# OpenResearchInstitute/opv-cxx-demod

Measured on AMD Instinct MI355X. Metric: IQ Msamples/s demod+Viterbi (×real-time @2.168MSPS); BER vs ref, higher is better.
Workload: dtype f64; 1 GPU; configs[3]: 64 concurrent IQ streams/GPU x 1000 frames, -s semantics, amp 2000, f0 -2000..+2000 Hz across the 64 streams of a shard (SURVEY.md §8d C4: edge streams on the AFC clamp, outside the +/-1530 Hz search span), Eb/N0 16 dB; streams_per_gpu=64, parallelism=streams sharded 64/GPU, no data-path collective

## Files before the change

### opv-cxx-demod_amd/csrc/k_frontend.hip

```cpp
#include <hip/hip_runtime.h>
#include <math.h>

#include <type_traits>

#include "k_frontend_common.h"

namespace {

constexpr uint32_t kTile = OPV_TILE_SAMPLES;
constexpr uint32_t kRing = 2 * kTile;
constexpr uint32_t kRingBytes = kRing * 4;
constexpr uint32_t kGuardBytes = 16;
constexpr uint32_t kBack = 11;
constexpr uint32_t kAhead = 56;
static_assert((kRing & (kRing - 1)) == 0, "ring must be a power of two");

constexpr uint32_t kTabOff = kRingBytes + kGuardBytes;
static_assert(kTabOff % 16 == 0, "16-byte LDS alignment");
constexpr uint32_t kAtanQBytes = 1025 * 32;
constexpr uintptr_t kRbLdsBase = 16;
static_assert(kRbLdsBase + kTabOff + kAtanQBytes == OPV_RB_LDS_I16, "launch size of the int16-ring shape");

constexpr uint32_t kF64Ring = 2048;
constexpr uint32_t kF64RingBytes = kF64Ring * 32;
constexpr uint32_t kF64Chunk = 256;
constexpr uint32_t kF64TabOff = 0;
constexpr uint32_t kF64RingOff = kAtanQBytes;
constexpr uint32_t kF64FlagOff = kF64RingOff + kF64RingBytes;
constexpr uint32_t kF64WaitSpins = 1u << 22;
constexpr uint32_t kHelperSpins = 1u << 22;
static_assert(kRbLdsBase + kF64FlagOff + 16 == OPV_RB_LDS_F64, "launch size of the fp64-ring shape");
static_assert(kF64Ring % kF64Chunk == 0 && (kF64Ring & (kF64Ring - 1)) == 0, "chunks tile the power-of-two ring");

typedef double d2v __attribute__((ext_vector_type(2)));
typedef __attribute__((address_space(3))) unsigned char lbyte;
typedef __attribute__((address_space(3))) int lint;
typedef __attribute__((address_space(3))) double ldouble;
typedef __attribute__((address_space(3))) d2v ld2v;

__device__ inline double swap32_add(double a, double b) {
    auto lo = __builtin_amdgcn_permlane32_swap((unsigned)dlo(a), (unsigned)dlo(b), false, false);
    auto hi = __builtin_amdgcn_permlane32_swap((unsigned)dhi(a), (unsigned)dhi(b), false, false);
    return mkd((int)hi[0], (int)lo[0]) + mkd((int)hi[1], (int)lo[1]);
}
__device__ inline double swap16_add(double a, double b) {
    auto lo = __builtin_amdgcn_permlane16_swap((unsigned)dlo(a), (unsigned)dlo(b), false, false);
    auto hi = __builtin_amdgcn_permlane16_swap((unsigned)dhi(a), (unsigned)dhi(b), false, false);
    return mkd((int)hi[0], (int)lo[0]) + mkd((int)hi[1], (int)lo[1]);
}
template <int N>
__device__ inline double row_bcast(double old, double v) { return __builtin_amdgcn_update_dpp(old, v, 0x150 + N, 0xF, 0xF, false); }
__device__ inline uint32_t uni(uint32_t v) { return (uint32_t)__builtin_amdgcn_readfirstlane((int)v); }
__device__ inline double readlane_d(double v, int l) {
    return mkd(__builtin_amdgcn_readlane(dhi(v), l), __builtin_amdgcn_readlane(dlo(v), l));
}
__device__ inline bool uni_lt(double a, double b) { return __builtin_amdgcn_fcmp(a, b, 4 ) != 0ull; }
__device__ inline bool uni_eq(double a, double b) { return __builtin_amdgcn_fcmp(a, b, 1 ) != 0ull; }

struct TagFirst { static constexpr bool first = true, wide = true; };
struct TagSecond { static constexpr bool first = false, wide = true; };
struct TagSteady { static constexpr bool first = false, wide = false; };

struct SinCosK {
    double s0, s1, s2, s3;
    double c0, c1, c2, c3, c4;
};
__device__ inline void expj_small(double kfs, double fo, const SinCosK& k, double& xs, double& xc) {
    double x, u, p, r, t;
    asm("v_mul_f64 %[x], %[kfs], %[fo]\n\t"
        "v_mul_f64 %[u], %[x], %[x]\n\t"
        "v_fma_f64 %[r], %[c4], %[u], %[c3]\n\t"
        "v_fma_f64 %[p], %[s3], %[u], %[s2]\n\t"
        "v_fma_f64 %[r], %[r], %[u], %[c2]\n\t"
        "v_fma_f64 %[p], %[p], %[u], %[s1]\n\t"
        "v_fma_f64 %[r], %[r], %[u], %[c1]\n\t"
        "v_fma_f64 %[p], %[p], %[u], %[s0]\n\t"
        "v_fma_f64 %[r], %[r], %[u], %[c0]\n\t"
        "v_mul_f64 %[t], %[x], %[u]\n\t"
        "v_fma_f64 %[xc], %[r], %[u], 1.0\n\t"
        "v_fma_f64 %[xs], %[t], %[p], %[x]"
        : [x] "=&v"(x), [u] "=&v"(u), [p] "=&v"(p), [r] "=&v"(r), [t] "=&v"(t), [xs] "=&v"(xs), [xc] "=&v"(xc)
        : [kfs] "v"(kfs), [fo] "v"(fo), [s0] "v"(k.s0), [s1] "v"(k.s1), [s2] "v"(k.s2), [s3] "v"(k.s3),
          [c0] "v"(k.c0), [c1] "v"(k.c1), [c2] "v"(k.c2), [c3] "v"(k.c3), [c4] "v"(k.c4));
}

}

#include "opv_atan2.h"

typedef __attribute__((address_space(3))) volatile uint32_t lds_flag;
__device__ inline lds_flag* f64_flags(lbyte* lds_all) {
    return reinterpret_cast<lds_flag*>(lds_all + kF64FlagOff);
}

__device__ void f64_ring_helper(const OpvStream& st, lbyte* lds_all) {
    const uint32_t lane = threadIdx.x & 63u;
    lds_flag* const fl = f64_flags(lds_all);
    const uint32_t n_avail = uni((uint32_t)st.n_avail), origin = uni((uint32_t)st.origin);
    const int* const iq = reinterpret_cast<const int*>(st.iq);
    uint32_t fill = ((origin >= kBack ? origin - kBack : 0u) / kF64Chunk) * kF64Chunk;
    const uint32_t fill_end = n_avail + kAhead + 2u;
    uint32_t spins = 0;
    while ((int)(fill - fill_end) < 0) {
        if (fl[2] != 0u) return;
        if ((int)(fl[0] + kF64Ring - fill - kF64Chunk) < 0) {
            if (++spins > kHelperSpins) return;
            __builtin_amdgcn_s_sleep(8);
            continue;
        }
        spins = 0;
        constexpr uint32_t kPerLane = kF64Chunk / 64u;
        const uint32_t n0 = fill + lane;
        int w[kPerLane], wn[kPerLane];
        if (fill + kF64Chunk < n_avail) {
#pragma unroll
            for (uint32_t k = 0; k < kPerLane; ++k) { w[k] = iq[n0 + 64u * k]; wn[k] = iq[n0 + 64u * k + 1u]; }
        } else {
#pragma unroll
            for (uint32_t k = 0; k < kPerLane; ++k) {
                const uint32_t n = n0 + 64u * k;
                w[k] = n < n_avail ? iq[n] : 0;
                wn[k] = n + 1u < n_avail ? iq[n + 1u] : 0;
            }
        }
#pragma unroll
        for (uint32_t k = 0; k < kPerLane; ++k) {
            const int xr = (int)(short)(w[k] & 0xFFFF), xi = w[k] >> 16;
            const int yr = (int)(short)(wn[k] & 0xFFFF) - xr, yi = (wn[k] >> 16) - xi;
            ld2v* e = reinterpret_cast<ld2v*>(lds_all + kF64RingOff + (((n0 + 64u * k) & (kF64Ring - 1u)) << 5));
            e[0] = d2v{(double)xr, (double)xi};
            e[1] = d2v{(double)yr, (double)yi};
        }
        __builtin_amdgcn_fence(__ATOMIC_RELEASE, "workgroup");
        fill += kF64Chunk;
        if (lane == 0u) fl[1] = fill;
    }
}

template <int WPB, bool F64 = false>
__device__ __forceinline__ void msk_frontend_body(OpvStream* __restrict__ streams, OpvGlobalCfg cfg, int n_streams,
                                                  lbyte* lds_all) {
    const int lane = threadIdx.x & 63;
    const int wave = WPB == 1 ? 0 : __builtin_amdgcn_readfirstlane((int)(threadIdx.x >> 6));
    const int sidx = (int)blockIdx.x * WPB + wave;
    const uint64_t dbg_t0 = __builtin_amdgcn_s_memtime(), dbg_r0 = __builtin_amdgcn_s_memrealtime();

    lbyte* const lds = lds_all + (F64 ? kF64RingOff : wave * kTabOff);
    const lbyte* ringb = lds;
    const ldouble* atab = reinterpret_cast<const ldouble*>(lds_all + (F64 ? kF64TabOff : WPB * kTabOff));
    if (sidx >= n_streams) return;
    OpvStream& st = streams[sidx];

    const int jsamp = lane - (lane >> 4) - ((lane & 15) == 15 ? 1 : 0);
    const double kf = (double)(jsamp - 10);
    const double kfs = kf * kDeltaPerHz;
    double wr[15], wi[15];
    {
        const int row = lane >> 4, t = lane & 15, u = t & 7;
        const bool is_p = u >= 6, imag = t >= 8;
        const int gate = (u < 2 || is_p) ? 1 : ((u & 1) ? 2 : 0);
        const bool tone2 = is_p ? false : (u < 2 ? u == 1 : u >= 4);
#pragma unroll
        for (int n = 0; n < 15; ++n) {
            const int i = 15 * row + n - 10 * gate;
            double sn, cs;
            sincospi((double)i / 80.0, &sn, &cs);
            const bool in = i >= 0 && i < 40;
            const double a = in ? cs : 0.0, b = in ? -sn : 0.0;
            double r_, i_;
            if (is_p) { r_ = (t == 6) ? a : (t == 15 ? b : 0.0); i_ = (t == 7) ? b : (t == 14 ? a : 0.0); }
            else if (!imag) { r_ = a; i_ = tone2 ? -b : b; }
            else { r_ = tone2 ? b : -b; i_ = a; }
            wr[n] = r_; wi[n] = i_;
            asm volatile("" : "+v"(wr[n]), "+v"(wi[n]));
        }
    }
    SinCosK sck;
    sck.s0 = -0x1.5555555555412p-3; sck.s1 = 0x1.1111110f26395p-7; sck.s2 = -0x1.a019e48059d90p-13; sck.s3 = 0x1.7150a543fadc5p-19;
    sck.c0 = -0x1.0000000000000p-1; sck.c1 = 0x1.5555555555014p-5; sck.c2 = -0x1.6c16c16818f3fp-10;
    sck.c3 = 0x1.a019dfaa26924p-16; sck.c4 = -0x1.276f06eab6283p-22;
    double kc_tfmax = 0.1, kc_beta = 0.00001, kc_alpha = 0.005, kc_fomax = 2000.0, kc_eps = 1e-10;
    double kc_tiny = 1e-100;
    asm volatile("" : "+v"(kc_tiny));
    double kc_halfpi = 1.57079632679489661923, kc_32 = 32.0, kc_m1_32 = -1.0 / 32.0, kc_gain = st.afc_alpha * (kSymRate / kTwoPi);
    [[maybe_unused]] double kc_64 = 512.0, kc_m1_64 = -1.0 / 512.0, kc_magic = 6755399441055744.0 + 512.0;
    asm volatile("" : "+v"(kc_64), "+v"(kc_m1_64), "+v"(kc_magic));
    asm volatile("" : "+v"(kc_tfmax), "+v"(kc_beta), "+v"(kc_alpha), "+v"(kc_fomax), "+v"(kc_eps));
    asm volatile("" : "+v"(kc_halfpi), "+v"(kc_32), "+v"(kc_m1_32), "+v"(kc_gain));
    const double kc_nfomax = __builtin_canonicalize(-kc_fomax), kc_ntfmax = __builtin_canonicalize(-kc_tfmax);
    kc_fomax = __builtin_canonicalize(kc_fomax);
    kc_tfmax = __builtin_canonicalize(kc_tfmax);
    double sx = 1.0, nsg = 1.0;
    asm volatile("" : "+v"(sx), "+v"(nsg));

    double fo = st.freq_offset, tf = st.timing_freq, mu = st.mu;
    PrevSums qp{st.p1r, st.p1i, st.p2r, st.p2i, st.x40c, st.x40s}, qq{0, 0, 0, 0, 1, 0};
    double fo_sum = st.fo_sum;
    uint32_t origin = uni((uint32_t)st.origin);
    const uint32_t n_avail = uni((uint32_t)st.n_avail);
    uint64_t n_soft = st.n_soft, total_samples = st.total_samples;
    uint32_t n_chunks = uni(st.n_chunks);
    int tail_done = (int)uni((uint32_t)st.tail_done);
    const int eof = (int)uni((uint32_t)st.eof);
    int overflow = (int)uni((uint32_t)st.overflow), stalled = 0;
    uint32_t edge_ties = uni(st.edge_ties);
    const uint64_t cap_soft = st.cap_soft;
    if (cap_soft > (1ull << 28)) overflow = 1;
    uint64_t soft_keep = st.trk_next >= 24 ? st.trk_next - 24 : 0;
    if (st.trk_state != 0 && st.trk_anchor < soft_keep) soft_keep = st.trk_anchor;
    const uint32_t soft_bmask = (uint32_t)(cap_soft * 8u - 1u) & ~7u;
    gbyte* const soft_base = (gbyte*)(((uint64_t)uni((uint32_t)((uint64_t)st.soft >> 32)) << 32) | uni((uint32_t)(uint64_t)st.soft));
    const gbyte* iq_bytes = (const gbyte*)st.iq;
    const uint64_t n_bytes = (uint64_t)n_avail * 4u;

    auto glds16 = [&](const gbyte* gsrc, uint32_t lds_byte) {
        unsigned keep;
        asm volatile("s_mov_b32 %0, m0\n\ts_mov_b32 m0, %2\n\ts_nop 0\n\tglobal_load_lds_dwordx4 %1, off\n\ts_mov_b32 m0, %0"
                     : "=&s"(keep)
                     : "v"(gsrc), "s"(uni(lds_byte))
                     : "memory");
    };
    const uint32_t lds_base = uni((uint32_t)(uintptr_t)lds);
    auto issue_tile = [&](uint32_t t) {
        const uint64_t base = (uint64_t)t * OPV_TILE_BYTES;
        const uint32_t slot = (t & 1u) * OPV_TILE_BYTES;
#pragma unroll
        for (int r = 0; r < 8; ++r) {
            const uint32_t in_tile = (uint32_t)r * 1024u + (uint32_t)lane * 16u;
            const uint64_t off = base + in_tile;
            if (off + 16u <= n_bytes) glds16(iq_bytes + off, lds_base + slot + (uint32_t)r * 1024u);
            else if (off < n_bytes) {
                for (uint32_t j = 0; off + 4u * j < n_bytes; ++j)
                    *reinterpret_cast<lint*>(lds + slot + in_tile + 4u * j) = *reinterpret_cast<const __attribute__((address_space(1))) int*>(iq_bytes + off + 4u * j);
            }
        }
        if ((t & 1u) == 0u && lane == 0) {
            if (base + 16u <= n_bytes) glds16(iq_bytes + base, lds_base + kRingBytes);
            else
                for (uint32_t j = 0; base + 4u * j < n_bytes && j < 4u; ++j)
                    *reinterpret_cast<lint*>(lds + kRingBytes + 4u * j) = *reinterpret_cast<const __attribute__((address_space(1))) int*>(iq_bytes + base + 4u * j);
        }
    };
    uint32_t t_lo = (origin >= kBack ? origin - kBack : 0u) / kTile;
    if constexpr (!F64) {
        issue_tile(t_lo);
        issue_tile(t_lo + 1u);
        __builtin_amdgcn_s_waitcnt(0x0F70);
    }
    bool evt_issue = true;
    uint32_t next_evt = (t_lo + 1u) * kTile + kBack;
    [[maybe_unused]] lds_flag* const fl = f64_flags(lds_all);
    [[maybe_unused]] auto f64_wait = [&](uint32_t need) {
        uint32_t r = uni(fl[1]);
        for (uint32_t spins = 0; (int)(r - need) < 0;) {
            if (overflow != 0 || ++spins > kF64WaitSpins) { overflow = 2; break; }
            __builtin_amdgcn_s_sleep(1);
            r = uni(fl[1]);
        }
        return r;
    };

    for (;;) {
        const uint32_t remaining = n_avail - origin;
        uint32_t N;
        bool last = false;
        if (cfg.streaming) {
            if (remaining >= OPV_CHUNK) N = OPV_CHUNK;
            else if (eof && !tail_done && remaining > 0) { N = remaining; last = true; }
            else { if (eof) tail_done = 1; break; }
        } else {
            if (!eof || tail_done) break;
            N = n_avail;
            last = true;
        }
        if (overflow) break;
        if ((n_soft - soft_keep) + (uint64_t)(N / 38u + 2u) > cap_soft) { stalled = 1; break; }

        const double Nd = (double)N;
        double pos = mu;
        const uint32_t soft_off0 = ((uint32_t)n_soft * 8u) & soft_bmask;
        uint32_t soft_off = soft_off0;
        asm volatile("" : "+v"(soft_off));

        auto housekeeping = [&](double at) {
            const uint32_t b = uni((uint32_t)at);
            const uint32_t gb = origin + b;
            if constexpr (F64) {
                if (lane == 0) fl[0] = gb >= kBack ? gb - kBack : 0u;
                uint32_t ready = uni(fl[1]);
                if ((int)(ready - gb) < (int)(kAhead + 2u)) ready = f64_wait(gb + kAhead + 2u);
                asm volatile("" ::: "memory");
                next_evt = ready - kAhead;
            }
            while (!F64 && gb >= next_evt) {
                if (evt_issue) {
                    issue_tile(t_lo + 2u);
                    ++t_lo;
                    evt_issue = false;
                    next_evt = (t_lo + 1u) * kTile - kAhead;
                } else {
                    __builtin_amdgcn_s_waitcnt(0x0F70);
                    evt_issue = true;
                    next_evt = (t_lo + 1u) * kTile + kBack;
                }
            }
            const int lim1 = (int)(next_evt - gb) - 2, lim2 = (int)N - 52 - (int)b;
            int lim = lim1 < lim2 ? lim1 : lim2;
            if (lim < 0) lim = 0;
            return ((uint32_t)lim * 1560u) >> 16;
        };

        int w0 = 0, w1 = 0;
        [[maybe_unused]] d2v x0{0.0, 0.0}, dx{0.0, 0.0};
        double f = 0.0;
        uint32_t tap_byte = 0;
        auto fetch_addr = [&](double at, bool clamp0) {
            double p = at + kf;
            if (clamp0) p = fmax(p, 0.0);
            const int idx = (int)p;
            f = __builtin_amdgcn_fract(p);
            if constexpr (F64) tap_byte = (((uint32_t)idx + origin) << 5) & (kF64RingBytes - 32u);
            else tap_byte = (((uint32_t)idx + origin) << 2) & (kRingBytes - 4u);
        };
        auto fetch_read = [&]() {
            if constexpr (F64) {
                const ld2v* tap = reinterpret_cast<const ld2v*>(ringb + tap_byte);
                x0 = tap[0];
                dx = tap[1];
            } else {
                const lint* tap = reinterpret_cast<const lint*>(ringb + tap_byte);
                w0 = tap[0];
                w1 = tap[1];
            }
        };
        auto fetch = [&](double at, bool clamp0) {
            fetch_addr(at, clamp0);
            fetch_read();
        };

        auto symbol_r = [&](auto tag, PrevSums& cur, const PrevSums& prv) {
            constexpr bool kFirst = decltype(tag)::first;
            constexpr bool kWide = decltype(tag)::wide;
            double xs, xc;
            if constexpr (kWide) {
                if (__builtin_expect(uni_lt(2000.0, fabs(fo)), 0)) sincos(kfs * fo, &xs, &xc);
                else expj_small(kfs, fo, sck, xs, xc);
            } else {
                expj_small(kfs, fo, sck, xs, xc);
            }
            __builtin_amdgcn_sched_barrier(0);
            const uint32_t my_soft_off = soft_off;
            uint32_t soft_off_next = soft_off + 8u;
            asm volatile("" : "+v"(soft_off_next));
            __builtin_amdgcn_sched_barrier(0);
            double lr, li;
            if constexpr (F64) {
                lr = fma(f, dx.x, x0.x);
                li = fma(f, dx.y, x0.y);
            } else {
                const int s0r = (int)(short)(w0 & 0xFFFF), s0i = w0 >> 16;
                const int d_r = (int)(short)(w1 & 0xFFFF) - s0r, d_i = (w1 >> 16) - s0i;
                lr = fma(f, (double)d_r, (double)s0r);
                li = fma(f, (double)d_i, (double)s0i);
            }
            const double zr = fma(lr, xc, li * xs);
            const double zi = fma(li, xc, -(lr * xs));
            __builtin_amdgcn_sched_barrier(0);

            double acc0, acc1, v, t;
#define OPV_RB(N) "v_fmac_f64_dpp %[a0], %[zr], %[r" #N "] row_newbcast:" #N " row_mask:0xf bank_mask:0xf\n\t" \
                  "v_fmac_f64_dpp %[a1], %[zi], %[i" #N "] row_newbcast:" #N " row_mask:0xf bank_mask:0xf\n\t"
            asm("v_mov_b64 %[a0], 0\n\tv_mov_b64 %[a1], 0\n\t" OPV_RB(0) OPV_RB(1) OPV_RB(2) OPV_RB(3) OPV_RB(4) OPV_RB(5) OPV_RB(6) OPV_RB(7)
                : [a0] "=&v"(acc0), [a1] "=&v"(acc1)
                : [zr] "v"(zr), [zi] "v"(zi), [r0] "v"(wr[0]), [i0] "v"(wi[0]), [r1] "v"(wr[1]), [i1] "v"(wi[1]), [r2] "v"(wr[2]), [i2] "v"(wi[2]),
                  [r3] "v"(wr[3]), [i3] "v"(wi[3]), [r4] "v"(wr[4]), [i4] "v"(wi[4]), [r5] "v"(wr[5]), [i5] "v"(wi[5]),
                  [r6] "v"(wr[6]), [i6] "v"(wi[6]), [r7] "v"(wr[7]), [i7] "v"(wi[7]));
            __builtin_amdgcn_sched_barrier(0);
            soft_off = soft_off_next & soft_bmask;
            asm volatile("" : "+v"(soft_off));
            __builtin_amdgcn_sched_barrier(0);
            asm(OPV_RB(8) OPV_RB(9) OPV_RB(10) OPV_RB(11) OPV_RB(12) OPV_RB(13) OPV_RB(14)
                "v_add_f64 %[v], %[a0], %[a1]\n\t"
                "v_mov_b64 %[t], %[v]"
                : [a0] "+v"(acc0), [a1] "+v"(acc1), [v] "=&v"(v), [t] "=&v"(t)
                : [zr] "v"(zr), [zi] "v"(zi), [r8] "v"(wr[8]), [i8] "v"(wi[8]), [r9] "v"(wr[9]), [i9] "v"(wi[9]), [r10] "v"(wr[10]), [i10] "v"(wi[10]),
                  [r11] "v"(wr[11]), [i11] "v"(wi[11]), [r12] "v"(wr[12]), [i12] "v"(wi[12]), [r13] "v"(wr[13]), [i13] "v"(wi[13]),
                  [r14] "v"(wr[14]), [i14] "v"(wi[14]));
#undef OPV_RB
            __builtin_amdgcn_sched_barrier(0);
            cur.x40c = readlane_d(xc, 53);
            __builtin_amdgcn_sched_barrier(0);
            v = swap32_add(v, t);
            asm("v_mov_b64 %0, %1" : "=v"(t) : "v"(v));
            __builtin_amdgcn_sched_barrier(0);
            cur.x40s = readlane_d(xs, 53);
            __builtin_amdgcn_sched_barrier(0);
            v = swap16_add(v, t);
            __builtin_amdgcn_sched_barrier(0);
            double fo_sum_next = fo_sum + fo;
            asm volatile("" : "+v"(fo_sum_next));
            const double sq = v * v;
            __builtin_amdgcn_sched_barrier(0);
            const double shv = mkd(__builtin_amdgcn_mov_dpp(dhi(v), 0x128, 0xF, 0xF, true), __builtin_amdgcn_mov_dpp(dlo(v), 0x128, 0xF, 0xF, true));
            const double en = fma(shv, shv, sq);
            __builtin_amdgcn_sched_barrier(0);
            const double P1o = row_bcast<6>(zr, v), P2o = row_bcast<7>(zi, v), P3o = row_bcast<14>(lr, v), P4o = row_bcast<15>(li, v);
            __builtin_amdgcn_sched_barrier(0);
            const double en1 = row_bcast<0>(acc0, en), en2 = row_bcast<1>(acc1, en);
            const double soft = en2 - en1;
            __builtin_amdgcn_sched_barrier(0);
            const bool dom1 = soft < 0.0;
            nsg = mkd((dhi(soft) & (int)0x80000000) | (dhi(nsg) & 0x7fffffff), dlo(nsg));
            asm volatile("" : "+v"(nsg));
            const double sg = -nsg;
            const double oth = mkd(__builtin_amdgcn_mov_dpp(dhi(en), 0x102, 0xF, 0xF, true), __builtin_amdgcn_mov_dpp(dlo(en), 0x102, 0xF, 0xF, true));
            __builtin_amdgcn_sched_barrier(0);
            double seln = dom1 ? en : oth;
            asm volatile("" : "+v"(seln));
            __builtin_amdgcn_sched_barrier(0);

            [[maybe_unused]] double pd = 0.0, cx = 0, cy = 0, sum = 1.0, dif = 0, dm_ = 1.0, ee, el;
            [[maybe_unused]] uint64_t zmask = 0;
            if constexpr (!kFirst) {
                const double dr = fma(sg, P2o, P1o), di = fma(-sg, P4o, P3o);
                const double prs = fma(sg, prv.a, prv.b), pis = fma(sg, prv.c, -prv.d);
                const double ar = fma(dr, prs, di * pis), ai = fma(di, prs, -(dr * pis));
                cy = fma(ar, prv.x40c, ai * prv.x40s);
                cx = fma(ar, prv.x40s, -(ai * prv.x40c));
                __builtin_amdgcn_sched_barrier(0);
                ee = row_bcast<2>(sq, seln); el = row_bcast<3>(shv, seln);
                __builtin_amdgcn_sched_barrier(0);
                sx = mkd((dhi(cx) & (int)0x80000000) | (dhi(sx) & 0x7fffffff), dlo(sx));
                asm volatile("" : "+v"(sx));
                sum = fabs(cx) + fabs(cy); dif = fabs(cy) - fabs(cx);
                dm_ = sum + kc_tiny;
                if constexpr (WPB == 1) {
                    zmask = __builtin_amdgcn_fcmp(sum, 0.0, 1 );
                    asm volatile("" : "+s"(zmask));
                }
            } else {
                ee = row_bcast<2>(sq, seln); el = row_bcast<3>(shv, seln);
            }
            const double den = el + ee + kc_eps;

            double ted, h = 0;
            [[maybe_unused]] d2v c01{0, 0}, c23{0, 0};
            if constexpr (kFirst) {
                double y = __builtin_amdgcn_rcp(den);
                const double num = el - ee;
                y = fma(fma(-den, y, 1.0), y, y);
                y = fma(fma(-den, y, 1.0), y, y);
                ted = num * y;
                ted = fma(fma(-den, ted, num), y, ted);
            } else {
                const double dm = dm_;
                const double tt = den * dm;
                double y = __builtin_amdgcn_rcp(tt);
                const double num = el - ee;
                y = fma(fma(-tt, y, 1.0), y, y);
                const double iden = y * dm, idm = y * den;
                const double ratio = dif * idm;
                const double kt = fma(ratio, kc_64, kc_magic);
                h = ratio;
                const lbyte* rowb = reinterpret_cast<const lbyte*>(atab) + ((unsigned)dlo(kt) << 5);
                const ld2v* trow = reinterpret_cast<const ld2v*>(rowb);
                c23 = trow[1]; c01 = trow[0];
                ted = num * iden;
                ted = fma(fma(-den, ted, num), iden, ted);
            }
            __builtin_amdgcn_sched_barrier(0);
            tf = clampd(fma(kc_beta, ted, tf), kc_ntfmax, kc_tfmax);
            const double adj = fma(kc_alpha, ted, tf);
            pos += 40.0 + adj;
            fetch_addr(pos, false);
            __builtin_amdgcn_sched_barrier(0);
            fetch_read();
            __builtin_amdgcn_sched_barrier(0);
            *(gdouble*)(soft_base + my_soft_off) = soft;
            if constexpr (!kFirst) {
                const double pd_off = fma(-sx, kc_halfpi, kc_halfpi);
                __builtin_amdgcn_sched_barrier(0);
                if constexpr (F64) __builtin_amdgcn_s_waitcnt(0xC27F);
                else __builtin_amdgcn_s_waitcnt(0xC17F);
                __builtin_amdgcn_sched_barrier(0);
                pd = fma(c23.y, h, c23.x);
                pd = fma(pd, h, c01.y);
                pd = fma(pd, h, c01.x);
                pd = fma(sx, pd, pd_off);
                pd = mkd((dhi(pd) & 0x7fffffff) | (dhi(cy) & (int)0x80000000), dlo(pd));
                if (__builtin_expect(WPB == 1 ? zmask != 0ull : uni_eq(sum, 0.0), 0)) {
                    const double dr = fma(sg, P2o, P1o), di = fma(-sg, P4o, P3o);
                    const double2 sp = silence_pd(dr, di, prv, soft < 0.0, fo_sum, n_soft + (((my_soft_off - soft_off0) & soft_bmask) >> 3),
                                                  P1o, P2o, P3o, P4o);
                    pd = sp.x;
                    edge_ties += uni((uint32_t)sp.y);
                }
                const double fo_new = fma(kc_gain, pd, fo);
                asm("v_max_f64 %0, %1, %2\n\tv_min_f64 %0, %0, %3" : "=&v"(fo) : "v"(fo_new), "v"(kc_nfomax), "v"(kc_fomax));
            }
            fo_sum = fo_sum_next;
            cur.a = P1o; cur.b = P2o; cur.c = P3o; cur.d = P4o;
        };

        auto sym = [&](auto tag, PrevSums& cur, const PrevSums& prv) { symbol_r(tag, cur, prv); };

        if (uni_lt(pos + 40.0 + 10.0, Nd)) {
            (void)housekeeping(pos);
            fetch(pos, true);
            sym(TagFirst{}, qp, qp);
            if (__builtin_expect(uni_lt(2000.0, fabs(fo)), 0) && uni_lt(pos + 40.0 + 10.0, Nd)) {
                (void)housekeeping(pos);
                fetch(pos, false);
                sym(TagSecond{}, qq, qp);
                qp = qq;
            }
            while (uni_lt(pos + 40.0 + 10.0, Nd)) {
                uint32_t pairs = uni(housekeeping(pos)) >> 1;
                if (F64 && overflow != 0) break;
                fetch(pos, false);
                for (uint32_t quads = pairs >> 1; quads != 0u; --quads) {
                    sym(TagSteady{}, qq, qp);
                    sym(TagSteady{}, qp, qq);
                    sym(TagSteady{}, qq, qp);
                    sym(TagSteady{}, qp, qq);
                }
                pairs &= 1u;
                for (; pairs != 0u; --pairs) {
                    sym(TagSteady{}, qq, qp);
                    sym(TagSteady{}, qp, qq);
                }
                sym(TagSteady{}, qq, qp);
                qp = qq;
            }
        }

        const uint32_t nsym_call = ((soft_off - soft_off0) & soft_bmask) >> 3;
        const uint32_t used = uni((uint32_t)pos);
        mu = pos - (double)used;
        const uint32_t leftover = N - used;
        if (lane == 0) {
            double* c = st.chunk_log + 5 * (size_t)(n_chunks % st.cap_chunks);
            c[0] = fo;
            c[1] = tf; c[2] = mu; c[3] = (double)leftover; c[4] = (double)nsym_call;
        }
        ++n_chunks;
        n_soft += nsym_call;
        total_samples += N;
        origin += (leftover > 0u && leftover < N) ? used : N;
        if (last) { tail_done = 1; break; }
    }

    if constexpr (F64) {
        if (lane == 0) fl[2] = 1u;
    }
    if (lane == 0) {
        st.freq_offset = fo;
        st.p1r = qp.a; st.p1i = qp.b; st.p2r = qp.c; st.p2i = qp.d; st.x40c = qp.x40c; st.x40s = qp.x40s;
        st.fo_sum = fo_sum;
        st.edge_ties = edge_ties;
        st.timing_freq = tf; st.mu = mu;
        st.origin = origin; st.n_soft = n_soft; st.total_samples = total_samples;
        st.n_chunks = n_chunks; st.tail_done = tail_done; st.overflow = overflow;
        st.stalled = stalled;
        unsigned hw, xcc;
        asm volatile("s_getreg_b32 %0, hwreg(HW_REG_HW_ID)" : "=s"(hw));
        asm volatile("s_getreg_b32 %0, hwreg(HW_REG_XCC_ID)" : "=s"(xcc));
        st.dbg_hw_id = hw; st.dbg_xcc_id = xcc;
        st.dbg_cycles = __builtin_amdgcn_s_memtime() - dbg_t0;
        st.dbg_ticks = __builtin_amdgcn_s_memrealtime() - dbg_r0;
    }
}

template <int NT>
__device__ __forceinline__ void load_atan_table_q(lbyte* lds_tab) {
    ldouble* atab = reinterpret_cast<ldouble*>(lds_tab);
    for (int i = threadIdx.x; i < 1025 * 4; i += NT) atab[i] = (&kOpvAtanTabQ3R[0][0])[i];
}
extern "C" __global__ __launch_bounds__(128) void k_msk_frontend_rb(OpvStream* __restrict__ streams, OpvGlobalCfg cfg,
                                                                     int n_streams) {
    lbyte* const lds_dyn = reinterpret_cast<lbyte*>(kRbLdsBase);
    if (blockDim.x == 128) {
        load_atan_table_q<128>(lds_dyn + kF64TabOff);
        if (threadIdx.x == 0) {
            __attribute__((address_space(3))) uint32_t* const fl = reinterpret_cast<__attribute__((address_space(3))) uint32_t*>(lds_dyn + kF64FlagOff);
            fl[0] = 0u;
            fl[1] = 0u;
            fl[2] = 0u;
        }
        __syncthreads();
        if (__builtin_amdgcn_readfirstlane((int)(threadIdx.x >> 6)) != 0) {
            if ((int)blockIdx.x < n_streams) f64_ring_helper(streams[blockIdx.x], lds_dyn);
            return;
        }
        msk_frontend_body<1, true>(streams, cfg, n_streams, lds_dyn);
    } else {
        load_atan_table_q<64>(lds_dyn + kTabOff);
        __syncthreads();
        msk_frontend_body<1>(streams, cfg, n_streams, lds_dyn);
    }
}
extern "C" __global__ __launch_bounds__(256) void k_msk_frontend_rb_wg4(OpvStream* __restrict__ streams, OpvGlobalCfg cfg,
                                                                         int n_streams) {
    __shared__ __attribute__((aligned(16))) unsigned char lds_all[4 * kTabOff + kAtanQBytes];
    lbyte* const lds = (lbyte*)lds_all;
    load_atan_table_q<256>(lds + 4 * kTabOff);
    __syncthreads();
    msk_frontend_body<4>(streams, cfg, n_streams, lds);
}
```

Baseline: 8841 Msamples/s.

## Trim per-symbol scalar and lane work in the f64 MSK frontend loop

Several micro-optimizations land together in the symbol loop. The soft-output offset now advances once per batch, with compile-time slot offsets and a ring-limit cap on batch size. The frequency clamp is folded into the next symbol's sincos asm. The readlane broadcasts of x40 become DPP row broadcasts, and the select of the dominant energy becomes a single DPP cndmask. Tap-address computation uses a mad_u16 with a precomputed ring base. The aim is fewer VALU/SALU ops and lane-to-scalar moves on the critical path, but it risks wrap and overflow subtleties in the 16-bit mad and changes to the jsamp mapping.

```diff
diff --git a/opv-cxx-demod_amd/csrc/k_frontend.hip b/opv-cxx-demod_amd/csrc/k_frontend.hip
--- a/opv-cxx-demod_amd/csrc/k_frontend.hip
+++ b/opv-cxx-demod_amd/csrc/k_frontend.hip
@@ -51,9 +51,6 @@
 template <int N>
 __device__ inline double row_bcast(double old, double v) { return __builtin_amdgcn_update_dpp(old, v, 0x150 + N, 0xF, 0xF, false); }
 __device__ inline uint32_t uni(uint32_t v) { return (uint32_t)__builtin_amdgcn_readfirstlane((int)v); }
-__device__ inline double readlane_d(double v, int l) {
-    return mkd(__builtin_amdgcn_readlane(dhi(v), l), __builtin_amdgcn_readlane(dlo(v), l));
-}
 __device__ inline bool uni_lt(double a, double b) { return __builtin_amdgcn_fcmp(a, b, 4 ) != 0ull; }
 __device__ inline bool uni_eq(double a, double b) { return __builtin_amdgcn_fcmp(a, b, 1 ) != 0ull; }
 
@@ -65,24 +62,36 @@
     double s0, s1, s2, s3;
     double c0, c1, c2, c3, c4;
 };
+#define OPV_EXPJ_ASM \
+    "v_mul_f64 %[x], %[kfs], %[fo]\n\t" \
+    "v_mul_f64 %[u], %[x], %[x]\n\t" \
+    "v_fma_f64 %[r], %[c4], %[u], %[c3]\n\t" \
+    "v_fma_f64 %[p], %[s3], %[u], %[s2]\n\t" \
+    "v_fma_f64 %[r], %[r], %[u], %[c2]\n\t" \
+    "v_fma_f64 %[p], %[p], %[u], %[s1]\n\t" \
+    "v_fma_f64 %[r], %[r], %[u], %[c1]\n\t" \
+    "v_fma_f64 %[p], %[p], %[u], %[s0]\n\t" \
+    "v_fma_f64 %[r], %[r], %[u], %[c0]\n\t" \
+    "v_mul_f64 %[t], %[x], %[u]\n\t" \
+    "v_fma_f64 %[xc], %[r], %[u], 1.0\n\t" \
+    "v_fma_f64 %[xs], %[t], %[p], %[x]"
 __device__ inline void expj_small(double kfs, double fo, const SinCosK& k, double& xs, double& xc) {
     double x, u, p, r, t;
-    asm("v_mul_f64 %[x], %[kfs], %[fo]\n\t"
-        "v_mul_f64 %[u], %[x], %[x]\n\t"
-        "v_fma_f64 %[r], %[c4], %[u], %[c3]\n\t"
-        "v_fma_f64 %[p], %[s3], %[u], %[s2]\n\t"
-        "v_fma_f64 %[r], %[r], %[u], %[c2]\n\t"
-        "v_fma_f64 %[p], %[p], %[u], %[s1]\n\t"
-        "v_fma_f64 %[r], %[r], %[u], %[c1]\n\t"
-        "v_fma_f64 %[p], %[p], %[u], %[s0]\n\t"
-        "v_fma_f64 %[r], %[r], %[u], %[c0]\n\t"
-        "v_mul_f64 %[t], %[x], %[u]\n\t"
-        "v_fma_f64 %[xc], %[r], %[u], 1.0\n\t"
-        "v_fma_f64 %[xs], %[t], %[p], %[x]"
+    asm(OPV_EXPJ_ASM
         : [x] "=&v"(x), [u] "=&v"(u), [p] "=&v"(p), [r] "=&v"(r), [t] "=&v"(t), [xs] "=&v"(xs), [xc] "=&v"(xc)
         : [kfs] "v"(kfs), [fo] "v"(fo), [s0] "v"(k.s0), [s1] "v"(k.s1), [s2] "v"(k.s2), [s3] "v"(k.s3),
           [c0] "v"(k.c0), [c1] "v"(k.c1), [c2] "v"(k.c2), [c3] "v"(k.c3), [c4] "v"(k.c4));
 }
+__device__ inline void expj_small_clamped(double kfs, double fo_raw, double fo_lo, double fo_hi, const SinCosK& k, double& fo,
+                                          double& xs, double& xc) {
+    double x, u, p, r, t;
+    asm("v_max_f64 %[fo], %[raw], %[lo]\n\t"
+        "v_min_f64 %[fo], %[fo], %[hi]\n\t" OPV_EXPJ_ASM
+        : [fo] "=&v"(fo), [x] "=&v"(x), [u] "=&v"(u), [p] "=&v"(p), [r] "=&v"(r), [t] "=&v"(t), [xs] "=&v"(xs), [xc] "=&v"(xc)
+        : [raw] "v"(fo_raw), [lo] "v"(fo_lo), [hi] "v"(fo_hi), [kfs] "v"(kfs), [s0] "v"(k.s0), [s1] "v"(k.s1), [s2] "v"(k.s2), [s3] "v"(k.s3),
+          [c0] "v"(k.c0), [c1] "v"(k.c1), [c2] "v"(k.c2), [c3] "v"(k.c3), [c4] "v"(k.c4));
+}
+#undef OPV_EXPJ_ASM
 
 }
 
@@ -151,7 +160,7 @@
     if (sidx >= n_streams) return;
     OpvStream& st = streams[sidx];
 
-    const int jsamp = lane - (lane >> 4) - ((lane & 15) == 15 ? 1 : 0);
+    const int jsamp = (lane & 15) == 15 ? 50 : lane - (lane >> 4);
     const double kf = (double)(jsamp - 10);
     const double kfs = kf * kDeltaPerHz;
     double wr[15], wi[15];
@@ -280,7 +289,15 @@
         double pos = mu;
         const uint32_t soft_off0 = ((uint32_t)n_soft * 8u) & soft_bmask;
         uint32_t soft_off = soft_off0;
-        asm volatile("" : "+v"(soft_off));
+        uint32_t soft_v = soft_off0;
+        asm volatile("" : "+v"(soft_v));
+        auto soft_advance = [&](uint32_t nsym) {
+            soft_off = (soft_off + 8u * nsym) & soft_bmask;
+            soft_v = soft_off;
+            asm volatile("" : "+v"(soft_v));
+        };
+        const uint32_t ring_c = (origin << 5) & (kF64RingBytes - 1u);
+        double fo_raw = fo;
 
         auto housekeeping = [&](double at) {
             const uint32_t b = uni((uint32_t)at);
@@ -307,7 +324,9 @@
             const int lim1 = (int)(next_evt - gb) - 2, lim2 = (int)N - 52 - (int)b;
             int lim = lim1 < lim2 ? lim1 : lim2;
             if (lim < 0) lim = 0;
-            return ((uint32_t)lim * 1560u) >> 16;
+            const uint32_t by_samples = ((uint32_t)lim * 1560u) >> 16;
+            const uint32_t by_ring = ((soft_bmask + 8u - soft_off) >> 3) - 1u;
+            return by_samples < by_ring ? by_samples : by_ring;
         };
 
         int w0 = 0, w1 = 0;
@@ -319,7 +338,7 @@
             if (clamp0) p = fmax(p, 0.0);
             const int idx = (int)p;
             f = __builtin_amdgcn_fract(p);
-            if constexpr (F64) tap_byte = (((uint32_t)idx + origin) << 5) & (kF64RingBytes - 32u);
+            if constexpr (F64) asm("v_mad_legacy_u16 %0, %1, 32, %2" : "+v"(tap_byte) : "v"(idx), "s"(ring_c));
             else tap_byte = (((uint32_t)idx + origin) << 2) & (kRingBytes - 4u);
         };
         auto fetch_read = [&]() {
@@ -338,20 +357,17 @@
             fetch_read();
         };
 
-        auto symbol_r = [&](auto tag, PrevSums& cur, const PrevSums& prv) {
+        auto symbol_r = [&](auto tag, auto slot, PrevSums& cur, const PrevSums& prv) {
             constexpr bool kFirst = decltype(tag)::first;
             constexpr bool kWide = decltype(tag)::wide;
+            constexpr uint32_t kSlot = decltype(slot)::value;
             double xs, xc;
             if constexpr (kWide) {
                 if (__builtin_expect(uni_lt(2000.0, fabs(fo)), 0)) sincos(kfs * fo, &xs, &xc);
                 else expj_small(kfs, fo, sck, xs, xc);
             } else {
-                expj_small(kfs, fo, sck, xs, xc);
-            }
-            __builtin_amdgcn_sched_barrier(0);
-            const uint32_t my_soft_off = soft_off;
-            uint32_t soft_off_next = soft_off + 8u;
-            asm volatile("" : "+v"(soft_off_next));
+                expj_small_clamped(kfs, fo_raw, kc_nfomax, kc_fomax, sck, fo, xs, xc);
+            }
             __builtin_amdgcn_sched_barrier(0);
             double lr, li;
             if constexpr (F64) {
@@ -371,29 +387,23 @@
 #define OPV_RB(N) "v_fmac_f64_dpp %[a0], %[zr], %[r" #N "] row_newbcast:" #N " row_mask:0xf bank_mask:0xf\n\t" \
                   "v_fmac_f64_dpp %[a1], %[zi], %[i" #N "] row_newbcast:" #N " row_mask:0xf bank_mask:0xf\n\t"
             asm("v_mov_b64 %[a0], 0\n\tv_mov_b64 %[a1], 0\n\t" OPV_RB(0) OPV_RB(1) OPV_RB(2) OPV_RB(3) OPV_RB(4) OPV_RB(5) OPV_RB(6) OPV_RB(7)
-                : [a0] "=&v"(acc0), [a1] "=&v"(acc1)
+                OPV_RB(8) OPV_RB(9) OPV_RB(10) OPV_RB(11) OPV_RB(12) OPV_RB(13) OPV_RB(14)
+                "v_add_f64 %[v], %[a0], %[a1]\n\t"
+                "v_mov_b64 %[t], %[v]"
+                : [a0] "=&v"(acc0), [a1] "=&v"(acc1), [v] "=&v"(v), [t] "=&v"(t)
                 : [zr] "v"(zr), [zi] "v"(zi), [r0] "v"(wr[0]), [i0] "v"(wi[0]), [r1] "v"(wr[1]), [i1] "v"(wi[1]), [r2] "v"(wr[2]), [i2] "v"(wi[2]),
                   [r3] "v"(wr[3]), [i3] "v"(wi[3]), [r4] "v"(wr[4]), [i4] "v"(wi[4]), [r5] "v"(wr[5]), [i5] "v"(wi[5]),
-                  [r6] "v"(wr[6]), [i6] "v"(wi[6]), [r7] "v"(wr[7]), [i7] "v"(wi[7]));
-            __builtin_amdgcn_sched_barrier(0);
-            soft_off = soft_off_next & soft_bmask;
-            asm volatile("" : "+v"(soft_off));
-            __builtin_amdgcn_sched_barrier(0);
-            asm(OPV_RB(8) OPV_RB(9) OPV_RB(10) OPV_RB(11) OPV_RB(12) OPV_RB(13) OPV_RB(14)
-                "v_add_f64 %[v], %[a0], %[a1]\n\t"
-                "v_mov_b64 %[t], %[v]"
-                : [a0] "+v"(acc0), [a1] "+v"(acc1), [v] "=&v"(v), [t] "=&v"(t)
-                : [zr] "v"(zr), [zi] "v"(zi), [r8] "v"(wr[8]), [i8] "v"(wi[8]), [r9] "v"(wr[9]), [i9] "v"(wi[9]), [r10] "v"(wr[10]), [i10] "v"(wi[10]),
+                  [r6] "v"(wr[6]), [i6] "v"(wi[6]), [r7] "v"(wr[7]), [i7] "v"(wi[7]),
+                  [r8] "v"(wr[8]), [i8] "v"(wi[8]), [r9] "v"(wr[9]), [i9] "v"(wi[9]), [r10] "v"(wr[10]), [i10] "v"(wi[10]),
                   [r11] "v"(wr[11]), [i11] "v"(wi[11]), [r12] "v"(wr[12]), [i12] "v"(wi[12]), [r13] "v"(wr[13]), [i13] "v"(wi[13]),
                   [r14] "v"(wr[14]), [i14] "v"(wi[14]));
 #undef OPV_RB
             __builtin_amdgcn_sched_barrier(0);
-            cur.x40c = readlane_d(xc, 53);
+            cur.x40c = row_bcast<15>(lr, xc);
+            cur.x40s = row_bcast<15>(li, xs);
             __builtin_amdgcn_sched_barrier(0);
             v = swap32_add(v, t);
             asm("v_mov_b64 %0, %1" : "=v"(t) : "v"(v));
-            __builtin_amdgcn_sched_barrier(0);
-            cur.x40s = readlane_d(xs, 53);
             __builtin_amdgcn_sched_barrier(0);
             v = swap16_add(v, t);
             __builtin_amdgcn_sched_barrier(0);
@@ -404,19 +414,26 @@
             const double shv = mkd(__builtin_amdgcn_mov_dpp(dhi(v), 0x128, 0xF, 0xF, true), __builtin_amdgcn_mov_dpp(dlo(v), 0x128, 0xF, 0xF, true));
             const double en = fma(shv, shv, sq);
             __builtin_amdgcn_sched_barrier(0);
-            const double P1o = row_bcast<6>(zr, v), P2o = row_bcast<7>(zi, v), P3o = row_bcast<14>(lr, v), P4o = row_bcast<15>(li, v);
+            const double P1o = row_bcast<6>(zr, v), P2o = row_bcast<7>(zi, v);
             __builtin_amdgcn_sched_barrier(0);
             const double en1 = row_bcast<0>(acc0, en), en2 = row_bcast<1>(acc1, en);
             const double soft = en2 - en1;
             __builtin_amdgcn_sched_barrier(0);
-            const bool dom1 = soft < 0.0;
+            double P3o, P4o;
+            int sel_lo, sel_hi;
+            asm("v_cmp_gt_f64 vcc, 0, %[soft]\n\t"
+                "v_mov_b64_dpp %[p3], %[v] row_newbcast:14 row_mask:0xf bank_mask:0xf\n\t"
+                "v_mov_b64_dpp %[p4], %[v] row_newbcast:15 row_mask:0xf bank_mask:0xf\n\t"
+                "v_cndmask_b32_dpp %[sl], %[el], %[el], vcc row_shl:2 row_mask:0xf bank_mask:0xf bound_ctrl:1\n\t"
+                "v_cndmask_b32_dpp %[sh], %[eh], %[eh], vcc row_shl:2 row_mask:0xf bank_mask:0xf bound_ctrl:1"
+                : [p3] "=&v"(P3o), [p4] "=&v"(P4o), [sl] "=&v"(sel_lo), [sh] "=&v"(sel_hi)
+                : [soft] "v"(soft), [v] "v"(v), [el] "v"(dlo(en)), [eh] "v"(dhi(en))
+                : "vcc");
+            const double seln = mkd(sel_hi, sel_lo);
+            __builtin_amdgcn_sched_barrier(0);
             nsg = mkd((dhi(soft) & (int)0x80000000) | (dhi(nsg) & 0x7fffffff), dlo(nsg));
             asm volatile("" : "+v"(nsg));
             const double sg = -nsg;
-            const double oth = mkd(__builtin_amdgcn_mov_dpp(dhi(en), 0x102, 0xF, 0xF, true), __builtin_amdgcn_mov_dpp(dlo(en), 0x102, 0xF, 0xF, true));
-            __builtin_amdgcn_sched_barrier(0);
-            double seln = dom1 ? en : oth;
-            asm volatile("" : "+v"(seln));
             __builtin_amdgcn_sched_barrier(0);
 
             [[maybe_unused]] double pd = 0.0, cx = 0, cy = 0, sum = 1.0, dif = 0, dm_ = 1.0, ee, el;
@@ -476,7 +493,7 @@
             __builtin_amdgcn_sched_barrier(0);
             fetch_read();
             __builtin_amdgcn_sched_barrier(0);
-            *(gdouble*)(soft_base + my_soft_off) = soft;
+            *(gdouble*)(soft_base + soft_v + 8u * kSlot) = soft;
             if constexpr (!kFirst) {
                 const double pd_off = fma(-sx, kc_halfpi, kc_halfpi);
                 __builtin_amdgcn_sched_barrier(0);
@@ -490,46 +507,61 @@
                 pd = mkd((dhi(pd) & 0x7fffffff) | (dhi(cy) & (int)0x80000000), dlo(pd));
                 if (__builtin_expect(WPB == 1 ? zmask != 0ull : uni_eq(sum, 0.0), 0)) {
                     const double dr = fma(sg, P2o, P1o), di = fma(-sg, P4o, P3o);
-                    const double2 sp = silence_pd(dr, di, prv, soft < 0.0, fo_sum, n_soft + (((my_soft_off - soft_off0) & soft_bmask) >> 3),
+                    const double2 sp = silence_pd(dr, di, prv, soft < 0.0, fo_sum, n_soft + (((soft_v + 8u * kSlot - soft_off0) & soft_bmask) >> 3),
                                                   P1o, P2o, P3o, P4o);
                     pd = sp.x;
                     edge_ties += uni((uint32_t)sp.y);
                 }
-                const double fo_new = fma(kc_gain, pd, fo);
-                asm("v_max_f64 %0, %1, %2\n\tv_min_f64 %0, %0, %3" : "=&v"(fo) : "v"(fo_new), "v"(kc_nfomax), "v"(kc_fomax));
+                fo_raw = fma(kc_gain, pd, fo);
             }
             fo_sum = fo_sum_next;
             cur.a = P1o; cur.b = P2o; cur.c = P3o; cur.d = P4o;
         };
 
-        auto sym = [&](auto tag, PrevSums& cur, const PrevSums& prv) { symbol_r(tag, cur, prv); };
+        auto fo_settle = [&]() {
+            asm("v_max_f64 %0, %1, %2\n\tv_min_f64 %0, %0, %3" : "=&v"(fo) : "v"(fo_raw), "v"(kc_nfomax), "v"(kc_fomax));
+            fo_raw = fo;
+        };
+        using Slot0 = std::integral_constant<uint32_t, 0>;
+        using Slot1 = std::integral_constant<uint32_t, 1>;
+        using Slot2 = std::integral_constant<uint32_t, 2>;
+        using Slot3 = std::integral_constant<uint32_t, 3>;
+        auto sym = [&](auto tag, auto slot, PrevSums& cur, const PrevSums& prv) { symbol_r(tag, slot, cur, prv); };
 
         if (uni_lt(pos + 40.0 + 10.0, Nd)) {
             (void)housekeeping(pos);
             fetch(pos, true);
-            sym(TagFirst{}, qp, qp);
+            sym(TagFirst{}, Slot0{}, qp, qp);
+            soft_advance(1u);
             if (__builtin_expect(uni_lt(2000.0, fabs(fo)), 0) && uni_lt(pos + 40.0 + 10.0, Nd)) {
                 (void)housekeeping(pos);
                 fetch(pos, false);
-                sym(TagSecond{}, qq, qp);
+                sym(TagSecond{}, Slot0{}, qq, qp);
+                fo_settle();
+                soft_advance(1u);
                 qp = qq;
             }
             while (uni_lt(pos + 40.0 + 10.0, Nd)) {
                 uint32_t pairs = uni(housekeeping(pos)) >> 1;
                 if (F64 && overflow != 0) break;
                 fetch(pos, false);
+                const uint32_t batch = 2u * pairs + 1u;
                 for (uint32_t quads = pairs >> 1; quads != 0u; --quads) {
-                    sym(TagSteady{}, qq, qp);
-                    sym(TagSteady{}, qp, qq);
-                    sym(TagSteady{}, qq, qp);
-                    sym(TagSteady{}, qp, qq);
+                    sym(TagSteady{}, Slot0{}, qq, qp);
+                    sym(TagSteady{}, Slot1{}, qp, qq);
+                    sym(TagSteady{}, Slot2{}, qq, qp);
+                    sym(TagSteady{}, Slot3{}, qp, qq);
+                    soft_v += 32u;
                 }
                 pairs &= 1u;
                 for (; pairs != 0u; --pairs) {
-                    sym(TagSteady{}, qq, qp);
-                    sym(TagSteady{}, qp, qq);
+                    sym(TagSteady{}, Slot0{}, qq, qp);
+                    sym(TagSteady{}, Slot1{}, qp, qq);
+                    soft_v += 16u;
                 }
-                sym(TagSteady{}, qq, qp);
+                sym(TagSteady{}, Slot0{}, qq, qp);
+                fo_settle();
+                soft_advance(batch);
                 qp = qq;
             }
         }
```

Measured after the change: 9153 Msamples/s, median of 6. +3.5%, better.
